# marsermd/DeepestScatter

Hardware: AMD Instinct MI355X
Metric: Msamples/s (rays x spp) at 512^3 vol, 1024^2 frame; HBM GB/s vs roofline (higher is better)
Workload: dtype f32

## Files before the change

### deepestscatter_amd/build.py

```python
from __future__ import annotations

import os
import shutil
import subprocess
import sys
from pathlib import Path

PKG = Path(__file__).resolve().parent
CSRC = PKG / "csrc"
ROOT = PKG.parent
LIB = PKG / "libcloudtrace.so"

SOURCES = ["ct_kernels.hip", "ct_group.hip", "ct_network.hip", "ct_api.cpp", "ct_host.cpp"]
HEADERS = [CSRC / "ct_device.hpp", CSRC / "ct_internal.hpp", CSRC / "ct_exchange.hpp", CSRC / "ct_sched.hpp", CSRC / "ct_network.hpp",
           ROOT / "include" / "cloudtrace.h",
           ROOT / "include" / "ct_fmath.h", PKG / "host" / "VdbReader.h"]

FLAGS = ["--offload-arch=gfx950", "-O3", "-std=c++17", "-ffp-contract=off", "-fno-fast-math", "-fno-slp-vectorize",
         "-fPIC", "-shared", "-fvisibility=hidden", "-Wall", "-Wno-unused-value"]


def hipcc() -> str:
    for cand in (os.environ.get("HIPCC"), shutil.which("hipcc"), "/opt/rocm/bin/hipcc"):
        if cand and Path(cand).exists():
            return cand
    raise RuntimeError("hipcc not found (need ROCm; set HIPCC=...)")


def needs_build() -> bool:
    if not LIB.exists():
        return True
    t = LIB.stat().st_mtime
    deps = [CSRC / s for s in SOURCES] + HEADERS
    return any(d.stat().st_mtime > t for d in deps)


HOST = PKG / "host"
CLI = HOST / "cloudtrace"


def build_cli(force: bool = False, verbose: bool = False) -> Path:
    srcs = [HOST / "main.cpp", HOST / "Cameras.h", HOST / "Scene.h", HOST / "SceneDescription.h", HOST / "VdbReader.h", HOST / "Collectors.h", HOST / "NetworkFile.h",
            ROOT / "include" / "cloudtrace.h"]
    if not force and CLI.exists() and LIB.exists() and all(s.stat().st_mtime <= CLI.stat().st_mtime for s in srcs + [LIB]):
        return CLI
    cmd = ["g++", "-std=c++17", "-O2", "-Wall", "-pthread", "-o", str(CLI), str(HOST / "main.cpp"), f"-L{PKG}", "-lcloudtrace",
           "-Wl,-rpath,$ORIGIN/.."]
    if verbose:
        print(" ".join(cmd), flush=True)
    subprocess.run(cmd, check=True)
    return CLI


VARIANTS = {
    "exp": ["-DCT_EXPERIMENTS"],
    "w8": ["-DCT_DELTA_THREADS=1024", "-DCT_DELTA_WAVES=8"],
    "nofuse": ["-DCT_DELTA_FUSE=0", "-DCT_MARCH_FUSE=0", "-DCT_DELTA_CHECK_EVERY=1"],
    "noendmerge": ["-DCT_DELTA_END_MERGE=0"],
    "noneeskip": ["-DCT_MARCH_NEE_SKIP=0"],
    "ab1": os.environ.get("CT_AB1_FLAGS", "").split(),
    "ab2": os.environ.get("CT_AB2_FLAGS", "").split(),
    "ab3": os.environ.get("CT_AB3_FLAGS", "").split(),
}


def build_variant(name: str, force: bool = False, verbose: bool = False) -> Path:
    out = PKG / f"libcloudtrace_{name}.so"
    deps = [CSRC / s for s in SOURCES] + HEADERS
    if force or not out.exists() or any(d.stat().st_mtime > out.stat().st_mtime for d in deps):
        cmd = [hipcc(), *FLAGS, *VARIANTS[name], "-o", str(out), *[str(CSRC / s) for s in SOURCES], "-lz", "-ldl"]
        if verbose:
            print(" ".join(cmd), flush=True)
        subprocess.run(cmd, check=True, cwd=str(CSRC))
    return out


def build(force: bool = False, verbose: bool = False) -> Path:
    if force or needs_build():
        cmd = [hipcc(), *FLAGS, *os.environ.get("CT_EXTRA_FLAGS", "").split(), "-o", str(LIB), *[str(CSRC / s) for s in SOURCES], "-lz", "-ldl"]
        if verbose:
            print(" ".join(cmd), flush=True)
        subprocess.run(cmd, check=True, cwd=str(CSRC))
    build_cli(force=force, verbose=verbose)
    return LIB


if __name__ == "__main__":
    if "--variant" in sys.argv:
        print(build_variant(sys.argv[sys.argv.index("--variant") + 1], force="--force" in sys.argv, verbose=True))
    else:
        print(build(force="--force" in sys.argv, verbose=True))
```

### deepestscatter_amd/cloudtrace.py

```python
from __future__ import annotations

import ctypes as C
from dataclasses import dataclass
from pathlib import Path

import numpy as np

from . import _lib
from ._lib import (CT_BUF_DENSITY, CT_BUF_FRAME, CT_BUF_INSCATTER, CT_BUF_M2, CT_BUF_MEAN, CT_BUF_SCREEN,
                   CtCounters, CtFetchCounters, CtScene, check)

MIE_FILE = Path(__file__).resolve().parent / "data" / "mie_raw.f32"

LIGHT_DIRECTIONS = {
    "Front": (-0.586, -0.766, -0.271),
    "Side": (-0.03, -0.25, 0.8),
    "Back": (0.586, -0.766, -0.271),
}


def load_mie_raw() -> tuple[np.ndarray, np.ndarray]:
    raw = np.fromfile(MIE_FILE, dtype="<f4")
    if raw.size != 8192:
        raise RuntimeError(f"{MIE_FILE} is corrupt")
# ... 484 lines not shown
        check(self.L.ct_debug_march_meta(self.h, _p(geom), C.c_void_p(), 0), self.h)
        d = {"radius": int(geom[0]), "bias_x": int(geom[1]), "bias": int(geom[2]),
             "bricks": tuple(int(v) for v in geom[3:6]), "sparse": bool(geom[6]), "meta": None}
        if not d["sparse"]:
            gx, gy, gz = d["bricks"]
            meta = np.zeros((gz * 4, gy * 4, gx), np.uint8)
            check(self.L.ct_debug_march_meta(self.h, _p(geom), _p(meta), meta.size), self.h)
            d["meta"] = meta
        return d

    LAYOUTS = ("density_bricks", "shadow_bricks", "march_bricks", "march_rows", "march_coarse", "twin_bricks", "majorant_cells",
               "majorant_codes", "mip_pyramid")

    def layout(self, which) -> tuple[np.ndarray, dict]:
        which = self.LAYOUTS.index(which) if isinstance(which, str) else int(which)
        geom, n = np.zeros(16, np.uint32), C.c_size_t(0)
        check(self.L.ct_debug_layout(self.h, which, _p(geom), C.c_void_p(), 0, C.byref(n)), self.h)
        g = [int(v) for v in geom]
        raw = np.zeros(n.value, np.uint8)
        check(self.L.ct_debug_layout(self.h, which, _p(geom), _p(raw), raw.size, C.byref(n)), self.h)
        if which in (_lib.CT_LAYOUT_DENSITY_BRICKS, _lib.CT_LAYOUT_SHADOW_BRICKS, _lib.CT_LAYOUT_TWIN_BRICKS):
            d = {"bias": g[0], "bricks": tuple(g[1:4])}
            return raw.reshape(g[3], g[2], g[1], 128), d
        if which == _lib.CT_LAYOUT_MARCH_BRICKS:
            d = {"bias_x": g[0], "bias": g[1], "bricks": tuple(g[2:5]), "sparse": bool(g[5])}
            return (raw.reshape(-1, 128) if d["sparse"] else raw.reshape(g[4], g[3], g[2], 128)), d
        if which == _lib.CT_LAYOUT_MARCH_ROWS:
            return raw.view(np.uint32).reshape(g[1], g[0], 2), {"rows": (g[0], g[1])}
        if which == _lib.CT_LAYOUT_MARCH_COARSE:
            return raw.reshape(g[3], g[2], g[1]), {"shift": g[0], "cells": tuple(g[1:4]), "bias": g[4]}
        if which == _lib.CT_LAYOUT_MIP_PYRAMID:
            return raw, {"levels": g[0], "dims": tuple(g[1:4])}
        d = {"cell": g[0], "div": g[1], "stored": tuple(g[2:5]), "origin": tuple(g[5:8]), "virtual": tuple(g[8:11]), "bias": g[11]}
        return raw.reshape(g[4], g[3], g[2]), d

    def kernel_time(self):
        a, b, n = C.c_double(0), C.c_double(0), C.c_uint64(0)
        check(self.L.ct_kernel_time(self.h, C.byref(a), C.byref(b), C.byref(n)), self.h)
        return float(a.value), float(b.value), int(n.value)

    def set_stream(self, hip_stream: int | None):
        check(self.L.ct_set_stream(self.h, C.c_void_p(hip_stream) if hip_stream else None), self.h)

    def debug_stats(self) -> dict:
        out = np.zeros(64, np.uint64)
        check(self.L.ct_debug_stats(self.h, _p(out)), self.h)
        names = ["regen_phases", "regen_lanes", "march_phases", "march_lanes", "scatter_phases", "scatter_lanes",
                 "fetched_steps", "fetched_zero_cells", "skipped_steps", "zero_cells_nonfree_brick",
                 "zero_cells_free_brick_d1", "skip_loop_wave_iterations", "nee_footprints_reused", "waves",
                 "stolen_jobs", "max_scheduler_visits_of_a_wave"]
        d = {n: int(v) for n, v in zip(names, out)}
        d["wave_end_hist_5ms"] = [int(v) for v in out[16:40]]
        d["wave_end_minus_drained_hist_0p5ms"] = [int(v) for v in out[40:64]]
        ex = np.zeros(73, np.uint64)
        check(self.L.ct_debug_stats_ex(self.h, _p(ex), 73), self.h)
        d["march_fetch_same_line_as_lanes_previous"] = int(ex[68])
        d["march_fetch_line_shared_with_a_lower_lane"] = int(ex[69])
        d["nee_lookups_skipped_shadow_zero"] = int(ex[72])
        d["raw"] = [int(v) for v in out]
        d["watchdog"] = int(out[63])
        return d

    def debug_suspended(self) -> int:
        n = C.c_uint64(0)
        check(self.L.ct_debug_suspended(self.h, C.byref(n)), self.h)
        return int(n.value)

    def debug_math_selftest(self, which: int) -> dict:
        out = np.zeros(3, np.uint64)
        check(self.L.ct_debug_math_selftest(self.h, which, _p(out)), self.h)
        return {"tested": int(out[0]), "mismatches": int(out[1]), "first_bad_bits": int(out[2])}

    def debug_cdf_inversion(self, first_u24: int, count: int) -> np.ndarray:
        out = np.empty(count, np.uint32)
        check(self.L.ct_debug_cdf_inversion(self.h, first_u24, count, _p(out)), self.h)
        return out


class TracerGroup:

    def __init__(self, density: np.ndarray, devices, params: SceneParams | None = None, **kw):
        self.L = _lib.load()
        self.params = params or SceneParams(**kw)
        s, keep = make_scene(density, self.params)
        self.width, self.height = self.params.width, self.params.height
        dev = np.asarray(list(devices), np.int32)
        g = C.c_void_p()
        rc = self.L.ct_group_create(C.byref(s), _p(dev), len(dev), C.byref(g))
        del keep
        if rc != _lib.CT_OK:
            msg = self.L.ct_group_last_error(None)
            raise _lib.CloudTraceError(rc, msg.decode("utf-8", "replace") if msg else "")
        self.g = g

    def _check(self, rc):
        if rc != _lib.CT_OK:
            msg = self.L.ct_group_last_error(self.g)
            raise _lib.CloudTraceError(rc, msg.decode("utf-8", "replace") if msg else "")

    def close(self):
        if getattr(self, "g", None):
            self.L.ct_group_destroy(self.g)
            self.g = None

    def __del__(self):
        try:
            self.close()
        except Exception:
            pass

    def set_camera(self, eye, U, V, W):
# ... 47 lines not shown
```

### deepestscatter_amd/csrc/ct_device.hpp

```cpp
#pragma once

#include <hip/hip_runtime.h>
#include <stdint.h>

#include "../../include/ct_fmath.h"

namespace ct {

#define CT_DEV __device__ __forceinline__

struct f3 {
    float x, y, z;
};

CT_DEV f3 mk3(float x, float y, float z) { return f3{ x, y, z }; }
CT_DEV f3 add3(f3 a, f3 b) { return mk3(a.x + b.x, a.y + b.y, a.z + b.z); }
CT_DEV f3 sub3(f3 a, f3 b) { return mk3(a.x - b.x, a.y - b.y, a.z - b.z); }
CT_DEV f3 scale3(f3 a, float s) { return mk3(a.x * s, a.y * s, a.z * s); }
CT_DEV float dot3(f3 a, f3 b) { return a.x * b.x + a.y * b.y + a.z * b.z; }
CT_DEV f3 cross3(f3 a, f3 b)
{
    return mk3(a.y * b.z - a.z * b.y, a.z * b.x - a.x * b.z, a.x * b.y - a.y * b.x);
}
CT_DEV float rcp_(float x) { return 1.0f / x; }
// ... 323 lines not shown
    const uint32_t bx = __umul24(ux, 43691u) >> 17, by = __umul24(uy, 43691u) >> 17, bz = __umul24(uz, 43691u) >> 17;
    const uint32_t lx = ux - __umul24(bx, 3u), ly = uy - __umul24(by, 3u), lz = uz - __umul24(bz, 3u);
    const uint32_t brick = __umul24(__umul24(bz, (uint32_t)sc.t_gy) + by, (uint32_t)sc.t_gx) + bx;
    const uint32_t local = (lz << 4) + (ly << 2) + lx;
#ifdef CT_DEBUG_BOUNDS
    if (bx >= (uint32_t)sc.t_gx || by >= (uint32_t)sc.t_gy || bz >= (uint32_t)sc.t_gz) {
        printf("CT_DEBUG_BOUNDS unclamped twin-brick texel (%u,%u,%u) outside the grid\n", ux, uy, uz);
        return 0;
    }
#endif
    return ((size_t)brick << 7) | local;
}
CT_DEV RawCell load_raw_twin(const uint8_t *q)
{
    RawCell r;
    __builtin_memcpy(&r.a, q, 8);
    __builtin_memcpy(&r.c, q + 14, 8);
    return r;
}
CT_DEV uint2 combine_twin(const RawCell &r)
{
    return make_uint2(__builtin_amdgcn_perm(r.a.y, r.a.x, 0x05040100u), __builtin_amdgcn_perm(r.c.y, r.c.x, 0x07060302u));
}

CT_DEV uint2 fetch_cell_cached(const DevScene &sc, const uint8_t *bricks, f3 p, uint32_t &key, uint2 &cached, bool &reused,
                               bool zero = false)
{
    const float fx = fmaf(p.x, sc.sx, -0.5f), fy = fmaf(p.y, sc.sy, -0.5f), fz = fmaf(p.z, sc.sz, -0.5f);
    const uint32_t x = (uint32_t)(floor_to_int(fx) + sc.brick_bias), y = (uint32_t)(floor_to_int(fy) + sc.brick_bias),
                   z = (uint32_t)(floor_to_int(fz) + sc.brick_bias);
    const uint32_t brick = __umul24(z >> 2, (uint32_t)sc.brick_gxy) + __umul24(y >> 2, (uint32_t)sc.brick_gx) + (x >> 2);
    const uint32_t local = __umul24(z & 3u, 25u) + __umul24(y & 3u, 5u) + (x & 3u);
    const uint32_t off = (brick << 7) | local;
    reused = sc.nee_cache != 0u && off == key;
    if (!reused && !zero) {
        const uint8_t *q = bricks + (((size_t)brick << 7) | local);
        uint2 a, c;
        __builtin_memcpy(&a, q, 8);
        __builtin_memcpy(&c, q + 25, 8);
        cached.x = __builtin_amdgcn_perm(a.y, a.x, 0x06050100u);
        cached.y = __builtin_amdgcn_perm(c.y, c.x, 0x06050100u);
        key = off;
    }
    return zero ? make_uint2(0u, 0u) : cached;
}

template <bool SPARSE>
CT_DEV uint2 fetch_cell_m(const DevScene &sc, f3 p, uint32_t &meta)
{
    const float x = fmaf(p.x, sc.sx, -0.5f), y = fmaf(p.y, sc.sy, -0.5f), z = fmaf(p.z, sc.sz, -0.5f);
    return load_footprint_m<SPARSE>(sc, floor_to_int(x), floor_to_int(y), floor_to_int(z), meta);
}

template <bool FIXED8>
CT_DEV float filter_at(const DevScene &sc, uint2 cell, f3 p)
{
    const float x = fmaf(p.x, sc.sx, -0.5f), y = fmaf(p.y, sc.sy, -0.5f), z = fmaf(p.z, sc.sz, -0.5f);
    return filter_cell(cell, tex_weight<FIXED8>(x), tex_weight<FIXED8>(y), tex_weight<FIXED8>(z));
}

template <bool FIXED8>
CT_DEV float tex3_clamped(const DevScene &sc, const uint8_t *bricks, f3 p)
{
    const float x = fmaf(p.x, sc.sx, -0.5f), y = fmaf(p.y, sc.sy, -0.5f), z = fmaf(p.z, sc.sz, -0.5f);
    const float flx = floorf(x), fly = floorf(y), flz = floorf(z);
    const int32_t ix = (int32_t)fminf(fmaxf(flx, -1.0f), (float)(sc.nx - 1));
    const int32_t iy = (int32_t)fminf(fmaxf(fly, -1.0f), (float)(sc.ny - 1));
    const int32_t iz = (int32_t)fminf(fmaxf(flz, -1.0f), (float)(sc.nz - 1));
    const uint2 c = load_footprint(sc, bricks, ix, iy, iz);
    return filter_cell(c, tex_weight<FIXED8>(x), tex_weight<FIXED8>(y), tex_weight<FIXED8>(z));
}

template <bool FIXED8, typename Ptr>
CT_DEV float tex1(Ptr t, float u)
{
    const float x = fmaf(u, (float)kMieN, -0.5f);
    const float fl = floorf(x);
    const int32_t i = (int32_t)fl;
    const int32_t i0 = min(max(i, 0), kMieN - 1);
    const int32_t i1 = min(max(i + 1, 0), kMieN - 1);
    const float a = t[i0], b = t[i1];
    return fmaf(tex_weight<FIXED8>(x), b - a, a);
}

template <typename CdfPtr, typename GuidePtr>
CT_DEV float sample_cos_theta(CdfPtr cdf, GuidePtr guide, uint32_t u24)
{
    const float val = u24_to_float(u24);
    const uint32_t bucket = u24 >> 12;
    uint32_t lo = guide[bucket], hi = guide[bucket + 1];
    while (lo < hi) {
        const uint32_t mid = (lo + hi) >> 1;
        if (cdf[mid] < val) {
            lo = mid + 1;
        } else {
            hi = mid;
        }
    }
    const uint32_t t = lo;
    uint32_t k = 0;
    if (t != 0) {
        const float a = cdf[t - 1];
        const float b = cdf[min(t, (uint32_t)kMieN - 1)];
        const float d = b - a;
        uint32_t s = 0;
#pragma unroll
// ... 95 lines not shown
```

### deepestscatter_amd/csrc/ct_internal.hpp

```cpp
#pragma once

#include <hip/hip_runtime.h>
#include <stdint.h>

#include "ct_device.hpp"

namespace ct {

constexpr int kTile = 8;
constexpr int kCounterCount = 9;
constexpr int kStatCount = 73;
constexpr int kContWords = 16;
constexpr int kContWordsDelta = 32;
constexpr int kLeftWords = 8;
constexpr int kQueueFlag = 32;
constexpr int kQueueDone = 16;
constexpr int kQueueWords = 64;
constexpr int kQueues = 8;

struct BatchArgs {
    float4 *frames;
    uint32_t frame_stride;
    const float4 *primary;
    const float4 *advance;
    const uint32_t *pixels;
    const uint32_t *group_rank;
    uint32_t rank_base;
    const uint32_t *job_group;
    const uint32_t *job_sub;
    uint2 *cost;
    uint32_t n_jobs;
    uint32_t q_begin[kQueues + 2];
    uint32_t reverse;
    uint32_t first_subframe;
    uint32_t S;
    uint32_t *queue;
    const uint32_t *cont_in;
    const uint32_t *cont_in_count;
    uint32_t *cont_cursor;
    uint32_t *cont_out;
    uint32_t *cont_out_count;
    uint32_t cont_capacity;
    uint32_t max_age;
    unsigned long long *cont_total;
    const uint32_t *left_in;
    const uint32_t *left_in_count;
    uint32_t *left_cursor;
    uint32_t *left_out;
    uint32_t *left_out_count;
    uint32_t left_capacity;
    uint32_t out_offset;
    unsigned long long *counters;
    unsigned long long *stats;
    unsigned long long *timeline;
    uint32_t *touched_density, *touched_shadow;
};

struct LaunchShape {
    int blocks;
    int threads;
    bool stats;
    uint32_t pool_slots = 0;
    uint32_t scatter_waves = 0;
};
// ... 126 lines not shown
```

### deepestscatter_amd/csrc/ct_kernels.hip

```cpp
#include <algorithm>
#include <cstdlib>

#include "ct_internal.hpp"

namespace ct {

__global__ void build_bricks_kernel(const uint8_t *__restrict__ t, int nx, int ny, int nz, int bias,
                                    uint8_t *__restrict__ bricks, int gx, int gy, int gz)
{
    const int64_t total = (int64_t)gx * gy * gz * 128;
    for (int64_t i = (int64_t)blockIdx.x * blockDim.x + threadIdx.x; i < total; i += (int64_t)gridDim.x * blockDim.x) {
        const int64_t b = i >> 7;
        const int o = (int)(i & 127);
        uint8_t v = 0;
        if (o < 125) {
            const int lx = o % 5, ly = (o / 5) % 5, lz = o / 25;
            const int x = (int)(b % gx) * 4 + lx - bias;
            const int y = (int)((b / gx) % gy) * 4 + ly - bias;
            const int z = (int)(b / ((int64_t)gx * gy)) * 4 + lz - bias;
            const int xc = min(max(x, 0), nx - 1), yc = min(max(y, 0), ny - 1), zc = min(max(z, 0), nz - 1);
            v = t[((size_t)zc * ny + yc) * nx + xc];
        }
        bricks[i] = v;
    }
// ... 835 lines not shown
    n.b = (i < 0) ? pair.x : pair.y;
    n.w = tex_weight<FIXED8>(x);
    n.cell = make_uint2(0u, 0u);
    return n;
}

template <bool FIXED8>
CT_DEV NeeLoads in_scattering_issue_lds(const DevScene &sc, const float *lds_chopped, f3 pos, f3 dir, bool chopped,
                                        uint32_t &nee_key, uint2 &nee_cell, bool &reused, bool zero = false)
{
    NeeLoads n;
    const float cos_light = dot3(mk3(sc.nlx, sc.nly, sc.nlz), dir);
    const float u = (cos_light + 1) / 2;
    const float x = fmaf(u, (float)kMieN, -0.5f);
    const int32_t i = (int32_t)floorf(x);
    const int32_t j = min(max(i, 0), kMieN - 2);
    float2 pair;
    if (chopped) {
        pair = make_float2(lds_chopped[j], lds_chopped[j + 1]);
    } else {
        __builtin_memcpy(&pair, sc.mie + j, sizeof pair);
    }
    n.a = (i > kMieN - 2) ? pair.y : pair.x;
    n.b = (i < 0) ? pair.x : pair.y;
    n.w = tex_weight<FIXED8>(x);
    n.cell = fetch_cell_cached(sc, sc.ibricks, pos, nee_key, nee_cell, reused, zero);
    return n;
}

template <bool FIXED8>
CT_DEV f3 in_scattering_finish(const DevScene &sc, const NeeLoads &n, f3 pos)
{
    const float phase = fmaf(n.w, n.b - n.a, n.a);
    const float ins = filter_at<FIXED8>(sc, n.cell, pos);
    f3 l = scale3(mk3(sc.lr, sc.lg, sc.lb), ins);
    l = scale3(l, phase);
    return scale3(l, sc.sun_ratio);
}

enum : int { ST_IDLE = 0, ST_MARCH = 1, ST_BOUNCE = 2 };

#ifndef CT_MARCH_FLAT_ZERO
#define CT_MARCH_FLAT_ZERO 1
#endif
#ifndef CT_MARCH_FLAT_EXIT
#define CT_MARCH_FLAT_EXIT 1
#endif
#ifndef CT_MARCH_FUSE
#define CT_MARCH_FUSE 1
#endif
constexpr bool MARCH_FUSE = CT_MARCH_FUSE != 0;
#ifndef CT_MARCH_NEE_SKIP
#define CT_MARCH_NEE_SKIP 1
#endif

CT_DEV float inv_max_advance(const DevScene &sc, f3 stepv)
{
    const float m = fmaxf(fmaxf(fabsf(stepv.x) * sc.sx, fabsf(stepv.y) * sc.sy), fabsf(stepv.z) * sc.sz);
    return __builtin_amdgcn_rcpf(fmaxf(m, 1e-20f));
}


CT_DEV int skip_steps(uint32_t c, float inv_maxd)
{
    return (int)(((float)c - 0.03125f) * inv_maxd);
}

CT_DEV void replay_steps(f3 &pos, f3 stepv, int n)
{
    int i = 0;
    for (; i + 8 <= n; i += 8) {
#pragma unroll
        for (int k = 0; k < 8; k++) {
            pos = add3(pos, stepv);
        }
    }
    for (; i < n; i++) {
        pos = add3(pos, stepv);
    }
}

template <bool FIXED8, bool SPARSE = false>
__global__ __launch_bounds__(256) void inscatter_kernel(DevScene sc, uint8_t *__restrict__ out, uint32_t zero_faces)
{
    const int64_t total = (int64_t)sc.nx * sc.ny * sc.nz;
    const int64_t i = (int64_t)blockIdx.x * blockDim.x + threadIdx.x;
    if (i >= total) {
        return;
    }
    const int x = (int)(i % sc.nx), y = (int)((i / sc.nx) % sc.ny), z = (int)(i / ((int64_t)sc.nx * sc.ny));
    const float max_size = (float)max(max(sc.nx, sc.ny), sc.nz);
    const float tsx = max_size / (float)sc.nx, tsy = max_size / (float)sc.ny, tsz = max_size / (float)sc.nz;
    const float min_scale = fminf(fminf(tsx, tsy), tsz);
    const float inv_min_scale = 1.0f / min_scale;
    f3 p = mk3((float)x / max_size, (float)y / max_size, (float)z / max_size);
    p = scale3(p, inv_min_scale);
    const f3 step_to_light = scale3(normalize3(mk3(sc.nlx, sc.nly, sc.nlz)), sc.sample_step);
    const int step_count = (int)(1 / sc.sample_step);
    float transmittance = 1;
    int s = 0;
    bool done = false;
    if (sc.mbricks != nullptr && (SPARSE || sc.m_rows == nullptr)) {
        const float inv_maxd = inv_max_advance(sc, step_to_light);
        while (s < step_count && in_box(sc, p)) {
            uint32_t meta;
            const uint2 cell = fetch_cell_m<SPARSE>(sc, p, meta);
// ... 95 lines not shown
            if ((cell.x | cell.y) != 0u || ((meta & 0x80u) == 0u && !in_box(sc, pos))) {
                break;
            }
        }
    }
    advance[p] = make_float4(start.x, start.y, start.z, __uint_as_float(start_bits));
}

hipError_t launch_primary_advance(const DevScene &sc, const float4 *primary, float4 *advance, hipStream_t stream)
{
    const dim3 grid((sc.width + 31) / 32, (sc.height + 7) / 8), block(256);
    if (sc.m_rows) {
        hipLaunchKernelGGL(primary_advance_kernel<true>, grid, block, 0, stream, sc, primary, advance);
    } else {
        hipLaunchKernelGGL(primary_advance_kernel<false>, grid, block, 0, stream, sc, primary, advance);
    }
    return hipGetLastError();
}

template <int MODE, bool STATS, bool SPARSE, bool COST = true, bool FIXED8 = false>
__global__ __launch_bounds__(512) __attribute__((amdgpu_waves_per_eu(6))) void render_persistent_kernel(DevScene sc, BatchArgs ba)
{
    __shared__ MieLdsFull lds;
    load_tables(sc, lds);

    const uint32_t lane = threadIdx.x & 63u;
#ifdef CT_DIAG_TIMELINE
    if (ba.timeline && lane == 0u) {
        ba.timeline[4u * (blockIdx.x * (blockDim.x >> 6) + (threadIdx.x >> 6))] = wall_clock64();
    }
#endif
    f3 pos = mk3(0, 0, 0), dir = mk3(0, 0, 1), stepv = mk3(0, 0, 0), rad = mk3(0, 0, 0);
    uint32_t seed = 0, depth = 0, out_idx = 0;
    uint32_t work = 0;
    float xi = 0, T = 1;
    uint32_t dfree = 0;
    float inv_maxd = 0;
    int state = ST_IDLE;

    JobState job{ 0, 0, 0, 0, 0, 0 };
    bool left_done = false;
    uint32_t q_cur = (uint32_t)kQueues, q_tried = 0;
    bool drained = false;
    uint32_t c_dl = 0, c_il = 0, c_cap = 0;
    uint32_t w_fetch = 0, w_nee = 0;
    uint32_t iv_dealt = 0, iv_written = 0, iv_resumed = 0, iv_suspended = 0;
    uint32_t nee_key = 0xffffffffu;
    uint2 nee_cell = make_uint2(0u, 0u);
    uint32_t st_regen = 0, st_regen_l = 0, st_march = 0, st_march_l = 0, st_scat = 0, st_scat_l = 0;
    uint32_t st_fetch = 0, st_zero = 0, st_skip = 0, st_zero_d0 = 0, st_zero_d1 = 0, st_skip_iters = 0, st_stolen = 0, st_iters = 0, st_first = 0;
    uint32_t st_hit2 = 0, st_hit3 = 0, st_h2 = 0xffffffffu, st_h3 = 0xffffffffu;
    uint32_t st_same_line = 0, st_dup_line = 0, st_prev_line = 0xffffffffu;
    uint32_t st_nee_zero = 0;

    uint32_t age = 0;
    if (ba.cont_in) {
        const uint32_t total = __builtin_amdgcn_readfirstlane(*ba.cont_in_count);
        uint32_t base = 0;
        if (lane == 0) {
            base = atomicAdd(ba.cont_cursor, 64u);
        }
        base = __builtin_amdgcn_readfirstlane(base);
        if (base + lane < total) {
            const uint4 *e = (const uint4 *)(ba.cont_in + (size_t)(base + lane) * kContWords);
            const uint4 w0 = e[0], w1 = e[1], w2 = e[2], w3 = e[3];
            pos = mk3(__uint_as_float(w0.x), __uint_as_float(w0.y), __uint_as_float(w0.z));
            dir = mk3(__uint_as_float(w0.w), __uint_as_float(w1.x), __uint_as_float(w1.y));
            rad = mk3(__uint_as_float(w1.z), __uint_as_float(w1.w), __uint_as_float(w2.x));
            seed = w2.y;
            out_idx = w2.z;
            xi = __uint_as_float(w2.w);
            T = __uint_as_float(w3.x);
            inv_maxd = __uint_as_float(w3.y);
            depth = w3.z & 0xffffu;
            dfree = (w3.z >> 16) & 0xffu;
            state = (int)(w3.z >> 24);
            stepv = scale3(dir, sc.sample_step);
            age = w3.w;
            if (STATS) {
                iv_resumed += 1;
            }
        }
    }
    const bool may_suspend = ba.cont_out != nullptr;
    const bool single_queue = ba.q_begin[1] == ba.n_jobs;

    const unsigned long long t_start = STATS ? wall_clock64() : 0ull;
    unsigned long long t_drained = 0;
#ifdef CT_DIAG_TIMELINE
    bool tl_marked = false;
#endif
    uint32_t visit = 0;
    for (;;) {
        visit += 1;
        if (may_suspend && single_queue && !drained && sc.hint_period != 0u && (visit & (sc.hint_period - 1u)) == 0u) {
            const uint32_t empty = __builtin_amdgcn_readfirstlane(__atomic_load_n(ba.queue + kQueueFlag, __ATOMIC_RELAXED));
            if (empty != 0u) {
                if (job.next != job.end && ba.left_out && job.age < ba.max_age && hand_on_job(ba, lane, job)) {
                    job.next = job.end;
                }
                if (job.next == job.end) {
                    drained = true;
                }
            }
        }
#ifdef CT_DIAG_TIMELINE
// ... 148 lines not shown
                    }
                    nee_fetched = !nee_reused && !nee_zero;
                    if (STATS) {
                        st_first += nee_reused ? 1u : 0u;
                        if (ba.touched_shadow && !nee_reused) {
                            const uint32_t line = (uint32_t)(apron_offset_in_grid(sc, pos) >> 7);
                            atomicOr(&ba.touched_shadow[line >> 5], 1u << (line & 31u));
                        }
                    }
                    c_il += 1;
                    if (COST) {
                        work += 4u;
                    }
                    bool go = (MODE != 2);
                    if (go) {
                        dir = new_direction(lds.cdf, lds.guide, seed, dir);
                        depth++;
                        if (depth == sc.max_depth) {
                            c_cap += 1;
                            go = false;
                        }
                    }
                    if (CT_MARCH_NEE_SKIP != 1 || !nee_zero) {
                        rad = add3(rad, in_scattering_finish<FIXED8>(sc, nee, pos));
                    }
                    if (go) {
                        xi = u24_to_float(lcg24(seed));
                        T = 1;
                        stepv = scale3(dir, sc.sample_step);
                        inv_maxd = inv_max_advance(sc, stepv);
                        dfree = 0;
                        state = ST_MARCH;
                    } else {
                        finished = true;
                    }
                } else {
                    finished = true;
                }
            }
            w_nee += (uint32_t)__builtin_popcountll(__builtin_amdgcn_ballot_w64(nee_fetched));
        }
        bool track = !do_scatter;
        uint32_t nm_track = nm;
        if (do_scatter && MARCH_FUSE) {
            nm_track = (uint32_t)__builtin_popcountll(__builtin_amdgcn_ballot_w64(state == ST_MARCH));
            track = nm_track != 0u;
        }
        if (track) {
            if (STATS) {
                st_march += 1;
                st_march_l += nm_track;
            }
            w_fetch += nm_track;
            uint32_t burst = drained ? sc.tail_burst : sc.march_burst;
            for (;;) {
            if (state == ST_MARCH) {
                if (dfree != 0u) {
                    const int n = skip_steps(dfree, inv_maxd);
                    replay_steps(pos, stepv, n);
                    c_dl += (uint32_t)n;
                    if (STATS) {
                        st_skip += (uint32_t)n;
                        int wmax = n;
#pragma unroll
                        for (int off = 32; off > 0; off >>= 1) {
                            wmax = max(wmax, __shfl_xor(wmax, off));
                        }
                        st_skip_iters += (lane_rank(__builtin_amdgcn_ballot_w64(true)) == 0u) ? (uint32_t)wmax : 0u;
                    }
                }
                pos = add3(pos, stepv);
                uint32_t meta;
                const uint2 cell = fetch_cell_m<SPARSE>(sc, pos, meta);
                dfree = meta & 0x3fu;
                c_dl += 1;
                if (COST) {
                    work += 1u;
                }
                if (STATS) {
                    st_fetch += 1;
                    {
                        const float fx = fmaf(pos.x, sc.sx, -0.5f), fy = fmaf(pos.y, sc.sy, -0.5f), fz = fmaf(pos.z, sc.sz, -0.5f);
                        const uint32_t lx = (uint32_t)(floor_to_int(fx) + sc.m_bias_x), ly = (uint32_t)(floor_to_int(fy) + sc.brick_bias),
                                       lz = (uint32_t)(floor_to_int(fz) + sc.brick_bias);
                        const uint32_t line = __umul24(lz >> 2, (uint32_t)sc.m_gxy) + __umul24(ly >> 2, (uint32_t)sc.m_gx) + (__umul24(lx, 43691u) >> 17);
                        st_same_line += (line == st_prev_line) ? 1u : 0u;
                        st_prev_line = line;
                        if (ba.touched_density && !SPARSE) {
                            atomicOr(&ba.touched_density[line >> 5], 1u << (line & 31u));
                        }
                        const uint64_t act = __builtin_amdgcn_ballot_w64(true);
                        bool dup = false;
                        for (uint32_t i = 0; i < 64u; i++) {
                            const uint32_t other = (uint32_t)__builtin_amdgcn_readlane((int)line, (int)i);
                            dup = dup || (((act >> i) & 1ull) != 0ull && i < lane && other == line);
                        }
                        st_dup_line += dup ? 1u : 0u;
                    }
                    st_zero += ((cell.x | cell.y) == 0u) ? 1u : 0u;
                    st_zero_d0 += ((cell.x | cell.y) == 0u && dfree == 0u) ? 1u : 0u;
                    st_zero_d1 += ((cell.x | cell.y) == 0u && dfree == 1u) ? 1u : 0u;
                }
                bool collided = false;
                if (CT_MARCH_FLAT_ZERO || (cell.x | cell.y) != 0u) {
                    const float density = filter_at<FIXED8>(sc, cell, pos) * sc.density_multiplier;
                    const float extinction = density * sc.sample_step;
                    T *= expf_inrange(-extinction);
                    if (xi > T) {
                        collided = true;
                        inv_maxd = density;
                    }
                }
#if CT_MARCH_FLAT_EXIT
                state = collided ? ST_BOUNCE : state;
                dfree = collided ? (meta & 0xc0u) : dfree;
                if (!collided & ((meta & 0x80u) == 0u) & !in_box_flat(sc, pos)) {
#else
                if (collided) {
                    state = ST_BOUNCE;
                    dfree = meta & 0xc0u;
                } else if ((meta & 0x80u) == 0u && !in_box(sc, pos)) {
#endif
                    ba.frames[out_idx] = make_float4(rad.x, rad.y, rad.z, 1.f);
                    if (STATS) {
                        iv_written += 1;
                    }
                    if (COST && ba.cost) {
                        ba.cost[out_idx - ba.out_offset] = make_uint2(work, depth);
                    }
                    state = ST_IDLE;
                }
            }
            if (--burst == 0u) {
                break;
            }
            const uint32_t m_now = (uint32_t)__builtin_popcountll(__builtin_amdgcn_ballot_w64(state == ST_MARCH));
            const uint32_t b_now = (uint32_t)__builtin_popcountll(__builtin_amdgcn_ballot_w64(state == ST_BOUNCE));
            if (drained) {
                if (m_now == 0u || 2u * b_now >= m_now + b_now) {
                    break;
                }
            } else if (m_now < sc.burst_march_min || b_now >= sc.burst_scatter || 64u - m_now - b_now >= sc.burst_idle) {
                break;
            }
            w_fetch += m_now;
            if (STATS) {
                st_march += 1;
                st_march_l += m_now;
            }
            }
        }
        if (finished) {
            ba.frames[out_idx] = make_float4(rad.x, rad.y, rad.z, 1.f);
            if (STATS) {
                iv_written += 1;
            }
            if (COST && ba.cost) {
                ba.cost[out_idx - ba.out_offset] = make_uint2(work, depth);
            }
            state = ST_IDLE;
        }
        if (may_suspend && drained && job.next == job.end) {
            const bool mine = state != ST_IDLE && age < ba.max_age;
            const uint64_t live = __builtin_amdgcn_ballot_w64(mine);
            if (live != 0ull) {
                const uint32_t n = (uint32_t)__builtin_popcountll(live);
                uint32_t base = 0;
                if (lane == (uint32_t)__builtin_ctzll(live)) {
                    base = atomicAdd(ba.cont_out_count, n);
                    if (base + n > ba.cont_capacity) {
                        atomicSub(ba.cont_out_count, n);
                        base = 0xffffffffu;
                    } else if (ba.cont_total) {
                        atomicAdd(ba.cont_total, (unsigned long long)n);
                    }
                }
                base = __builtin_amdgcn_readlane(base, __builtin_ctzll(live));
                if (mine && base != 0xffffffffu) {
                    uint4 *e = (uint4 *)(ba.cont_out + (size_t)(base + lane_rank(live)) * kContWords);
                    e[0] = make_uint4(__float_as_uint(pos.x), __float_as_uint(pos.y), __float_as_uint(pos.z), __float_as_uint(dir.x));
                    e[1] = make_uint4(__float_as_uint(dir.y), __float_as_uint(dir.z), __float_as_uint(rad.x), __float_as_uint(rad.y));
                    e[2] = make_uint4(__float_as_uint(rad.z), seed, out_idx, __float_as_uint(xi));
                    e[3] = make_uint4(__float_as_uint(T), __float_as_uint(inv_maxd), depth | (dfree << 16) | ((uint32_t)state << 24), age + 1u);
                    state = ST_IDLE;
                    if (STATS) {
                        iv_suspended += 1;
                    }
                }
            }
        }
    }

#ifdef CT_DIAG_TIMELINE
    if (ba.timeline && lane == 0u) {
        ba.timeline[4u * (blockIdx.x * (blockDim.x >> 6) + (threadIdx.x >> 6)) + 1u] = wall_clock64();
    }
#endif
    const uint32_t vals[3] = { wave_sum(c_dl), wave_sum(c_il), wave_sum(c_cap) };
    if (STATS) {
        uint32_t sv[16] = { st_fetch, st_zero, st_skip, st_zero_d0, st_zero_d1, st_skip_iters, st_first,
                            iv_dealt, iv_resumed, iv_written, iv_suspended, st_same_line, st_dup_line, st_hit2, st_hit3, st_nee_zero };
#pragma unroll
        for (int i = 0; i < 16; i++) {
            sv[i] = wave_sum(sv[i]);
        }
        if (lane == 0) {
            atomicAdd(&ba.stats[0], (unsigned long long)st_regen);
            atomicAdd(&ba.stats[1], (unsigned long long)st_regen_l);
            atomicAdd(&ba.stats[2], (unsigned long long)st_march);
            atomicAdd(&ba.stats[3], (unsigned long long)st_march_l);
            atomicAdd(&ba.stats[4], (unsigned long long)st_scat);
            atomicAdd(&ba.stats[5], (unsigned long long)st_scat_l);
            atomicAdd(&ba.stats[6], (unsigned long long)sv[0]);
            atomicAdd(&ba.stats[7], (unsigned long long)sv[1]);
            atomicAdd(&ba.stats[8], (unsigned long long)sv[2]);
            atomicAdd(&ba.stats[9], (unsigned long long)sv[3]);
            atomicAdd(&ba.stats[10], (unsigned long long)sv[4]);
            atomicAdd(&ba.stats[11], (unsigned long long)sv[5]);
            atomicAdd(&ba.stats[12], (unsigned long long)sv[6]);
            atomicAdd(&ba.stats[13], 1ull);
            atomicAdd(&ba.stats[14], (unsigned long long)st_stolen);
            atomicMax(&ba.stats[15], (unsigned long long)st_iters);
            const unsigned long long t_end = wall_clock64();
#ifdef CT_STATS_FINE
            atomicAdd(&ba.stats[16 + min((unsigned long long)23, (t_end - t_start) / 25000ull)], 1ull);
            atomicAdd(&ba.stats[40 + min((unsigned long long)23, (t_end - (t_drained ? t_drained : t_end)) / 5000ull)], 1ull);
#else
            atomicAdd(&ba.stats[16 + min((unsigned long long)23, (t_end - t_start) / 500000ull)], 1ull);
            atomicAdd(&ba.stats[40 + min((unsigned long long)23, (t_end - (t_drained ? t_drained : t_end)) / 50000ull)], 1ull);
#endif
            atomicAdd(&ba.stats[64], (unsigned long long)sv[7]);
            atomicAdd(&ba.stats[65], (unsigned long long)sv[8]);
            atomicAdd(&ba.stats[66], (unsigned long long)sv[9]);
            atomicAdd(&ba.stats[67], (unsigned long long)sv[10]);
            atomicAdd(&ba.stats[68], (unsigned long long)sv[11]);
            atomicAdd(&ba.stats[69], (unsigned long long)sv[12]);
            atomicAdd(&ba.stats[70], (unsigned long long)sv[13]);
            atomicAdd(&ba.stats[71], (unsigned long long)sv[14]);
            atomicAdd(&ba.stats[72], (unsigned long long)sv[15]);
        }
    }
    flush_counters(ba, lane, vals[0], vals[1], vals[2], w_fetch, w_nee);
}

__global__ void mip_level_kernel(const uint8_t *__restrict__ prev, int px, int py, int pz, uint8_t *__restrict__ cur,
                                 int cx, int cy, int cz)
{
    const int64_t total = (int64_t)cx * cy * cz;
    for (int64_t i = (int64_t)blockIdx.x * blockDim.x + threadIdx.x; i < total; i += (int64_t)gridDim.x * blockDim.x) {
        const int x = (int)(i % cx), y = (int)((i / cx) % cy), z = (int)(i / ((int64_t)cx * cy));
        uint32_t acc = 0;
#pragma unroll
        for (int d = 0; d < 8; d++) {
            const int sx = 2 * x + (d & 1), sy = 2 * y + ((d >> 1) & 1), sz = 2 * z + (d >> 2);
            if (sx < px && sy < py && sz < pz) {
                acc += prev[((size_t)sz * py + sy) * px + sx];
            }
        }
        cur[i] = (uint8_t)(acc / 8u);
    }
}

hipError_t launch_mip_level(const uint8_t *prev, int px, int py, int pz, uint8_t *cur, int cx, int cy, int cz,
                            hipStream_t stream)
{
    const int64_t total = (int64_t)cx * cy * cz;
    const int blocks = (int)std::min<int64_t>((total + 255) / 256, 65536);
    hipLaunchKernelGGL(mip_level_kernel, dim3(blocks), dim3(256), 0, stream, prev, px, py, pz, cur, cx, cy, cz);
    return hipGetLastError();
}

template <bool FIXED8>
CT_DEV float tex3_level(const DevScene &sc, const MipPyramid &mp, uint32_t l, f3 p)
{
    const int32_t nx = mp.nx[l], ny = mp.ny[l], nz = mp.nz[l];
    const float x = fmaf(p.x, sc.tsx * (float)nx, -0.5f), y = fmaf(p.y, sc.tsy * (float)ny, -0.5f),
                z = fmaf(p.z, sc.tsz * (float)nz, -0.5f);
    const float flx = floorf(x), fly = floorf(y), flz = floorf(z);
    const float wx = tex_weight<FIXED8>(x), wy = tex_weight<FIXED8>(y), wz = tex_weight<FIXED8>(z);
    const int32_t ix = (int32_t)flx, iy = (int32_t)fly, iz = (int32_t)flz;
    const int32_t x0 = min(max(ix, 0), nx - 1), x1 = min(max(ix + 1, 0), nx - 1);
    const int32_t y0 = min(max(iy, 0), ny - 1), y1 = min(max(iy + 1, 0), ny - 1);
    const int32_t z0 = min(max(iz, 0), nz - 1), z1 = min(max(iz + 1, 0), nz - 1);
    const uint8_t *b = mp.base + mp.offset[l];
    const size_t sy_ = (size_t)nx, sz_ = (size_t)nx * (size_t)ny;
    uint2 c;
    c.x = (uint32_t)b[z0 * sz_ + y0 * sy_ + x0] | ((uint32_t)b[z0 * sz_ + y0 * sy_ + x1] << 8) |
          ((uint32_t)b[z0 * sz_ + y1 * sy_ + x0] << 16) | ((uint32_t)b[z0 * sz_ + y1 * sy_ + x1] << 24);
    c.y = (uint32_t)b[z1 * sz_ + y0 * sy_ + x0] | ((uint32_t)b[z1 * sz_ + y0 * sy_ + x1] << 8) |
          ((uint32_t)b[z1 * sz_ + y1 * sy_ + x0] << 16) | ((uint32_t)b[z1 * sz_ + y1 * sy_ + x1] << 24);
    return filter_cell(c, wx, wy, wz);
}
// ... 1734 lines not shown
```

Measured before the change: 3670.

## Pair march steps by issuing both density footprint loads before evaluating

In the dense march loop, the footprint for the next step is loaded together with the current one, with the second position clamped to the grid, so two memory requests are in flight at once. If the first step stays in ST_MARCH, needs no empty-space skip and the clamped position was in range, the second step is evaluated from the prefetched data and the burst counter drops by one extra. This is meant to hide latency of the dependent per-step loads. In exchange it wastes a load whenever the second step is dropped, and it adds register pressure, which the code tries to limit by packing depth and age into one register. New stats counters track paired and dropped steps.

```diff
diff --git a/deepestscatter_amd/build.py b/deepestscatter_amd/build.py
--- a/deepestscatter_amd/build.py
+++ b/deepestscatter_amd/build.py
@@ -58,6 +58,7 @@
     "nofuse": ["-DCT_DELTA_FUSE=0", "-DCT_MARCH_FUSE=0", "-DCT_DELTA_CHECK_EVERY=1"],
     "noendmerge": ["-DCT_DELTA_END_MERGE=0"],
     "noneeskip": ["-DCT_MARCH_NEE_SKIP=0"],
+    "nopair": ["-DCT_MARCH_PAIR=0"],
     "ab1": os.environ.get("CT_AB1_FLAGS", "").split(),
     "ab2": os.environ.get("CT_AB2_FLAGS", "").split(),
     "ab3": os.environ.get("CT_AB3_FLAGS", "").split(),
diff --git a/deepestscatter_amd/cloudtrace.py b/deepestscatter_amd/cloudtrace.py
--- a/deepestscatter_amd/cloudtrace.py
+++ b/deepestscatter_amd/cloudtrace.py
@@ -560,11 +560,13 @@
         d = {n: int(v) for n, v in zip(names, out)}
         d["wave_end_hist_5ms"] = [int(v) for v in out[16:40]]
         d["wave_end_minus_drained_hist_0p5ms"] = [int(v) for v in out[40:64]]
-        ex = np.zeros(73, np.uint64)
-        check(self.L.ct_debug_stats_ex(self.h, _p(ex), 73), self.h)
+        ex = np.zeros(75, np.uint64)
+        check(self.L.ct_debug_stats_ex(self.h, _p(ex), 75), self.h)
         d["march_fetch_same_line_as_lanes_previous"] = int(ex[68])
         d["march_fetch_line_shared_with_a_lower_lane"] = int(ex[69])
         d["nee_lookups_skipped_shadow_zero"] = int(ex[72])
+        d["march_second_steps"] = int(ex[73])
+        d["march_prefetches_dropped"] = int(ex[74])
         d["raw"] = [int(v) for v in out]
         d["watchdog"] = int(out[63])
         return d
diff --git a/deepestscatter_amd/csrc/ct_device.hpp b/deepestscatter_amd/csrc/ct_device.hpp
--- a/deepestscatter_amd/csrc/ct_device.hpp
+++ b/deepestscatter_amd/csrc/ct_device.hpp
@@ -399,6 +399,69 @@
     return load_footprint_m<SPARSE>(sc, floor_to_int(x), floor_to_int(y), floor_to_int(z), meta);
 }
 
+struct FootprintPair {
+    uint2 a1, c1;
+    uint32_t lx1;
+    uint2 a2, c2;
+    bool ok;
+};
+CT_DEV FootprintPair request_footprint_pair_m(const DevScene &sc, f3 p1, f3 p2)
+{
+    FootprintPair f;
+    uint32_t brick1, local1, brick2, local2;
+    {
+        const int32_t ix = floor_to_int(fmaf(p1.x, sc.sx, -0.5f)), iy = floor_to_int(fmaf(p1.y, sc.sy, -0.5f)),
+                      iz = floor_to_int(fmaf(p1.z, sc.sz, -0.5f));
+        const uint32_t x = (uint32_t)(ix + sc.m_bias_x), y = (uint32_t)(iy + sc.brick_bias), z = (uint32_t)(iz + sc.brick_bias);
+        const uint32_t bx = __umul24(x, 43691u) >> 17;
+        const uint32_t lx = x - __umul24(bx, 3u);
+        uint32_t brick = __umul24(z >> 2, (uint32_t)sc.m_gxy) + __umul24(y >> 2, (uint32_t)sc.m_gx) + bx;
+        uint32_t local = __umul24(z & 3u, 25u) + __umul24(y & 3u, 5u) + lx;
+#ifdef CT_DEBUG_BOUNDS
+        if (bx >= (uint32_t)sc.m_gx || (y >> 2) >= (uint32_t)sc.brick_gy || (z >> 2) >= (uint32_t)sc.brick_gz) {
+            printf("CT_DEBUG_BOUNDS march-brick texel (%d,%d,%d) outside the grid\n", ix, iy, iz);
+            brick = local = 0u;
+        }
+#endif
+        brick1 = brick;
+        local1 = local;
+        f.lx1 = lx;
+    }
+    {
+        const int32_t ux = floor_to_int(fmaf(p2.x, sc.sx, -0.5f)) + sc.m_bias_x, uy = floor_to_int(fmaf(p2.y, sc.sy, -0.5f)) + sc.brick_bias,
+                      uz = floor_to_int(fmaf(p2.z, sc.sz, -0.5f)) + sc.brick_bias;
+        const int32_t xmax = min(3 * sc.m_gx, 1 << 17) - 1;
+        const int32_t cx = min(max(ux, 0), xmax), cy = min(max(uy, 0), 4 * sc.brick_gy - 1), cz = min(max(uz, 0), 4 * sc.brick_gz - 1);
+        const uint32_t x = (uint32_t)cx, y = (uint32_t)cy, z = (uint32_t)cz;
+        const uint32_t bx = __umul24(x, 43691u) >> 17;
+        const uint32_t lx = x - __umul24(bx, 3u);
+        const uint32_t brick = __umul24(z >> 2, (uint32_t)sc.m_gxy) + __umul24(y >> 2, (uint32_t)sc.m_gx) + bx;
+        const uint32_t local = __umul24(z & 3u, 25u) + __umul24(y & 3u, 5u) + lx;
+        brick2 = brick;
+        local2 = local;
+        f.ok = (cx == ux) & (cy == uy) & (cz == uz);
+    }
+    asm volatile("" : "+v"(brick1), "+v"(brick2));
+    const uint8_t *q1 = sc.mbricks + (((size_t)brick1 << 7) | local1), *q2 = sc.mbricks + (((size_t)brick2 << 7) | local2);
+    __builtin_memcpy(&f.a1, q1, 8);
+    __builtin_memcpy(&f.c1, q1 + 25, 8);
+    __builtin_memcpy(&f.a2, q2, 8);
+    __builtin_memcpy(&f.c2, q2 + 25, 8);
+    return f;
+}
+CT_DEV uint2 finish_footprint_first(const FootprintPair &f, uint32_t &meta)
+{
+    meta = __builtin_amdgcn_perm(f.a1.y, f.a1.x, 0x0c0c0c04u - f.lx1);
+    return make_uint2(__builtin_amdgcn_perm(f.a1.y, f.a1.x, 0x06050100u), __builtin_amdgcn_perm(f.c1.y, f.c1.x, 0x06050100u));
+}
+CT_DEV uint2 finish_footprint_ahead(const DevScene &sc, const FootprintPair &f, f3 p, uint32_t &meta)
+{
+    const uint32_t x = (uint32_t)(floor_to_int(fmaf(p.x, sc.sx, -0.5f)) + sc.m_bias_x);
+    const uint32_t lx = x - __umul24(__umul24(x, 43691u) >> 17, 3u);
+    meta = __builtin_amdgcn_perm(f.a2.y, f.a2.x, 0x0c0c0c04u - lx);
+    return make_uint2(__builtin_amdgcn_perm(f.a2.y, f.a2.x, 0x06050100u), __builtin_amdgcn_perm(f.c2.y, f.c2.x, 0x06050100u));
+}
+
 template <bool FIXED8>
 CT_DEV float filter_at(const DevScene &sc, uint2 cell, f3 p)
 {
diff --git a/deepestscatter_amd/csrc/ct_internal.hpp b/deepestscatter_amd/csrc/ct_internal.hpp
--- a/deepestscatter_amd/csrc/ct_internal.hpp
+++ b/deepestscatter_amd/csrc/ct_internal.hpp
@@ -9,7 +9,7 @@
 
 constexpr int kTile = 8;
 constexpr int kCounterCount = 9;
-constexpr int kStatCount = 73;
+constexpr int kStatCount = 75;
 constexpr int kContWords = 16;
 constexpr int kContWordsDelta = 32;
 constexpr int kLeftWords = 8;
diff --git a/deepestscatter_amd/csrc/ct_kernels.hip b/deepestscatter_amd/csrc/ct_kernels.hip
--- a/deepestscatter_amd/csrc/ct_kernels.hip
+++ b/deepestscatter_amd/csrc/ct_kernels.hip
@@ -911,6 +911,9 @@
 constexpr bool MARCH_FUSE = CT_MARCH_FUSE != 0;
 #ifndef CT_MARCH_NEE_SKIP
 #define CT_MARCH_NEE_SKIP 1
+#endif
+#ifndef CT_MARCH_PAIR
+#define CT_MARCH_PAIR 1
 #endif
 
 CT_DEV float inv_max_advance(const DevScene &sc, f3 stepv)
@@ -1112,6 +1115,7 @@
     uint32_t st_hit2 = 0, st_hit3 = 0, st_h2 = 0xffffffffu, st_h3 = 0xffffffffu;
     uint32_t st_same_line = 0, st_dup_line = 0, st_prev_line = 0xffffffffu;
     uint32_t st_nee_zero = 0;
+    uint32_t st_second = 0, st_dropped = 0;
 
     uint32_t age = 0;
     if (ba.cont_in) {
@@ -1366,26 +1370,14 @@
                 st_march_l += nm_track;
             }
             w_fetch += nm_track;
-            uint32_t burst = drained ? sc.tail_burst : sc.march_burst;
-            for (;;) {
-            if (state == ST_MARCH) {
-                if (dfree != 0u) {
-                    const int n = skip_steps(dfree, inv_maxd);
-                    replay_steps(pos, stepv, n);
-                    c_dl += (uint32_t)n;
-                    if (STATS) {
-                        st_skip += (uint32_t)n;
-                        int wmax = n;
-#pragma unroll
-                        for (int off = 32; off > 0; off >>= 1) {
-                            wmax = max(wmax, __shfl_xor(wmax, off));
-                        }
-                        st_skip_iters += (lane_rank(__builtin_amdgcn_ballot_w64(true)) == 0u) ? (uint32_t)wmax : 0u;
-                    }
-                }
-                pos = add3(pos, stepv);
-                uint32_t meta;
-                const uint2 cell = fetch_cell_m<SPARSE>(sc, pos, meta);
+#if CT_MARCH_PAIR
+            uint32_t depth_age = depth | (age << 16);
+            asm volatile("" : "+v"(depth_age));
+#define CT_BURST_DEPTH (depth_age & 0xffffu)
+#else
+#define CT_BURST_DEPTH depth
+#endif
+            auto eval_step = [&](const uint2 cell, const uint32_t meta) {
                 dfree = meta & 0x3fu;
                 c_dl += 1;
                 if (COST) {
@@ -1435,16 +1427,80 @@
                     dfree = meta & 0xc0u;
                 } else if ((meta & 0x80u) == 0u && !in_box(sc, pos)) {
 #endif
+#if CT_MARCH_PAIR
+                    asm volatile("" : "+v"(out_idx));
+#endif
                     ba.frames[out_idx] = make_float4(rad.x, rad.y, rad.z, 1.f);
                     if (STATS) {
                         iv_written += 1;
                     }
                     if (COST && ba.cost) {
-                        ba.cost[out_idx - ba.out_offset] = make_uint2(work, depth);
+                        ba.cost[out_idx - ba.out_offset] = make_uint2(work, CT_BURST_DEPTH);
                     }
                     state = ST_IDLE;
                 }
-            }
+            };
+            uint32_t burst = drained ? sc.tail_burst : sc.march_burst;
+            for (;;) {
+#if CT_MARCH_PAIR
+            const bool pair = !SPARSE && burst >= 2u;
+            bool second = false;
+#endif
+            if (state == ST_MARCH) {
+                if (dfree != 0u) {
+                    const int n = skip_steps(dfree, inv_maxd);
+                    replay_steps(pos, stepv, n);
+                    c_dl += (uint32_t)n;
+                    if (STATS) {
+                        st_skip += (uint32_t)n;
+                        int wmax = n;
+#pragma unroll
+                        for (int off = 32; off > 0; off >>= 1) {
+                            wmax = max(wmax, __shfl_xor(wmax, off));
+                        }
+                        st_skip_iters += (lane_rank(__builtin_amdgcn_ballot_w64(true)) == 0u) ? (uint32_t)wmax : 0u;
+                    }
+                }
+                pos = add3(pos, stepv);
+#if CT_MARCH_PAIR
+                if (pair) {
+                    const FootprintPair fp = request_footprint_pair_m(sc, pos, add3(pos, stepv));
+                    uint32_t meta;
+                    const uint2 cell = finish_footprint_first(fp, meta);
+                    eval_step(cell, meta);
+                    if ((state == ST_MARCH) & fp.ok && skip_steps(dfree, inv_maxd) == 0) {
+                        second = true;
+                        asm volatile("" : "+v"(pos.x), "+v"(pos.y), "+v"(pos.z));
+                        pos = add3(pos, stepv);
+                        uint32_t meta2;
+                        const uint2 cell2 = finish_footprint_ahead(sc, fp, pos, meta2);
+                        eval_step(cell2, meta2);
+                    }
+                    if (STATS) {
+                        st_second += second ? 1u : 0u;
+                        st_dropped += second ? 0u : 1u;
+                    }
+                } else
+#endif
+                {
+                    uint32_t meta;
+                    const uint2 cell = fetch_cell_m<SPARSE>(sc, pos, meta);
+                    eval_step(cell, meta);
+                }
+            }
+#if CT_MARCH_PAIR
+            {
+                const uint32_t n_second = (uint32_t)__builtin_popcountll(__builtin_amdgcn_ballot_w64(second));
+                w_fetch += n_second;
+                if (n_second != 0u) {
+                    burst -= 1u;
+                    if (STATS) {
+                        st_march += 1;
+                        st_march_l += n_second;
+                    }
+                }
+            }
+#endif
             if (--burst == 0u) {
                 break;
             }
@@ -1463,6 +1519,12 @@
                 st_march_l += m_now;
             }
             }
+#if CT_MARCH_PAIR
+            asm volatile("" : "+v"(depth_age));
+            depth = depth_age & 0xffffu;
+            age = depth_age >> 16;
+#endif
+#undef CT_BURST_DEPTH
         }
         if (finished) {
             ba.frames[out_idx] = make_float4(rad.x, rad.y, rad.z, 1.f);
@@ -1512,10 +1574,11 @@
 #endif
     const uint32_t vals[3] = { wave_sum(c_dl), wave_sum(c_il), wave_sum(c_cap) };
     if (STATS) {
-        uint32_t sv[16] = { st_fetch, st_zero, st_skip, st_zero_d0, st_zero_d1, st_skip_iters, st_first,
-                            iv_dealt, iv_resumed, iv_written, iv_suspended, st_same_line, st_dup_line, st_hit2, st_hit3, st_nee_zero };
+        uint32_t sv[18] = { st_fetch, st_zero, st_skip, st_zero_d0, st_zero_d1, st_skip_iters, st_first,
+                            iv_dealt, iv_resumed, iv_written, iv_suspended, st_same_line, st_dup_line, st_hit2, st_hit3, st_nee_zero,
+                            st_second, st_dropped };
 #pragma unroll
-        for (int i = 0; i < 16; i++) {
+        for (int i = 0; i < 18; i++) {
             sv[i] = wave_sum(sv[i]);
         }
         if (lane == 0) {
@@ -1552,6 +1615,8 @@
             atomicAdd(&ba.stats[70], (unsigned long long)sv[13]);
             atomicAdd(&ba.stats[71], (unsigned long long)sv[14]);
             atomicAdd(&ba.stats[72], (unsigned long long)sv[15]);
+            atomicAdd(&ba.stats[73], (unsigned long long)sv[16]);
+            atomicAdd(&ba.stats[74], (unsigned long long)sv[17]);
         }
     }
     flush_counters(ba, lane, vals[0], vals[1], vals[2], w_fetch, w_nee);
```

Result: slower. 3498 (-4.7%).
